# hammershock/SFM-Python

Hardware: AMD Instinct MI355X
Metric: BA iterations/sec (higher is better)
Workload: dtype f64

## Files before the change

### sfm-python_amd/csrc/ba_kernels.hpp

```cpp
#pragma once

#include <hip/hip_runtime.h>
#include <stdint.h>

#include "tr2d.hpp"

namespace sfmba {

constexpr int kCamTab = 17;
constexpr int kCamRow = 18;
#ifndef SFMBA_REC_LAYOUT
#define SFMBA_REC_LAYOUT 0
#endif
constexpr int kRecLayout = SFMBA_REC_LAYOUT;
constexpr int kRec = kRecLayout == 0 ? 6 : (kRecLayout == 1 ? 8 : 16);
constexpr int kVinvRow = kRecLayout == 0 ? 6 : (kRecLayout == 1 ? 8 : 16);
constexpr int kVinvInRec = kRecLayout == 2 ? 8 : -1;
constexpr int kRhsRec = 16;
constexpr int kSweepThreads = 1024;
constexpr int kWavesPerSweepBlock = kSweepThreads / 64;

struct KMat { double k[9]; };

constexpr int kJPlanes = 6;
// ... 1026 lines not shown
                }
            }
#pragma unroll
            for (int u = 0; u < kScalePts; ++u) {
                const int p = p0 + u * (int)blockDim.x;
                if (p >= P) continue;
#pragma unroll
                for (int k = 0; k < 3; ++k) {
                    double s, sge;
                    element(d[u][k], ge[u][k], so[u][k], xe[u][k], s, sge);
                    sip[(size_t)p * 3 + k] = s; gpo[(size_t)p * 3 + k] = ge[u][k]; sgp[(size_t)p * 3 + k] = sge;
                }
            }
        }
    }
    write_partials(q, part);
}


__global__ void k_post(Mailbox mb) { post_mailbox(mb); }

__global__ void k_finish(const double* __restrict__ part, FinishJob job, int nq, int first_sum,
                         double* __restrict__ out, const double* __restrict__ skip, Mailbox mb) {
    if (skip != nullptr && *skip != 0.0) {
        if (mb.host != nullptr && blockIdx.x == 0 && threadIdx.x < 64) post_mailbox(mb);
        return;
    }
    const int k = threadIdx.x >> 6;
    if (k < nq) finish_task(part, job, (int)blockIdx.x, k, nq, first_sum, out);
    if (mb.host != nullptr) {
        __syncthreads();
        if (threadIdx.x < 64) post_mailbox(mb);
    }
}

struct Recompute {
    const double* __restrict__ camtab;
    const double* __restrict__ pts;
    KMat K;
};
__device__ __forceinline__ void stage_cam_table(const double* __restrict__ camtab, int C, double* __restrict__ smem) {
    const int n2 = (C * kCamRow) >> 1;
    const double2* __restrict__ src = reinterpret_cast<const double2*>(camtab);
    double2* __restrict__ dst = reinterpret_cast<double2*>(smem);
    for (int k = threadIdx.x; k < n2; k += blockDim.x) dst[k] = src[k];
    __syncthreads();
}
__device__ __forceinline__ void recompute_blocks(const Recompute& rc, const double* __restrict__ tab_lds, int c, int p,
                                                 double* jc, double* jp) {
    double tl[kCamRow];
    const double2* __restrict__ trow = reinterpret_cast<const double2*>(tab_lds + (size_t)c * kCamRow);
#pragma unroll
    for (int k = 0; k < kCamRow / 2; ++k) { const double2 q = trow[k]; tl[2 * k] = q.x; tl[2 * k + 1] = q.y; }
    const double* __restrict__ Xp = rc.pts + 3 * (size_t)p;
    double rx, ry;
    observe<true>(tl, Xp[0], Xp[1], Xp[2], 0.0, 0.0, rc.K, rx, ry, jc, jp);
}

template <bool LDS_VEC, bool JFREE = false>
__global__ __launch_bounds__(kSweepThreads) void k_jdot(ObsArrays o, const double* __restrict__ sgc,
                                                        const double* __restrict__ sgp, int N, int C,
                                                        double* __restrict__ t1,
                                                        double* __restrict__ part, Piggyback pb, Recompute rc) {
    static_assert(!(LDS_VEC && JFREE), "J-free: the LDS holds the camera table, the vector comes from L2");
    extern __shared__ __align__(16) double smem[];
    __shared__ double red[kWavesPerSweepBlock];
// ... 2398 lines not shown
```

### sfm-python_amd/csrc/sfmba.hip

```cpp
#include "../../include/sfmba.h"

#include <hip/hip_runtime.h>
#include <hip/hip_ext.h>
#include <rccl/rccl.h>
#include <dlfcn.h>

#include <algorithm>
#include <atomic>
#include <chrono>
#include <cmath>
#include <cstdarg>
#include <cstdio>
#include <cstdlib>
#include <cstring>
#include <condition_variable>
#include <functional>
#include <mutex>
#include <numeric>
#include <string>
#include <thread>
#include <vector>

#include "ba_kernels.hpp"
#include "tr2d.hpp"
// ... 13 lines not shown
    void* p = nullptr;
    size_t bytes = 0;
    ~DevBuf() { if (p) (void)hipFree(p); }
    hipError_t ensure(size_t n) {
        if (n <= bytes && p) return hipSuccess;
        if (p) { (void)hipFree(p); p = nullptr; bytes = 0; }
        if (n == 0) n = 8;
        hipError_t e = hipMalloc(&p, n);
        if (e == hipSuccess) bytes = n;
        return e;
    }
    hipError_t ensure_keep(size_t n, size_t keep) {
        if (n <= bytes && p) return hipSuccess;
        if (keep == 0 || !p) return ensure(n + n / 2);
        void* q = nullptr;
        const size_t cap = n + n / 2;
        hipError_t e = hipMalloc(&q, cap);
        if (e != hipSuccess) return e;
        e = hipMemcpy(q, p, std::min(keep, bytes), hipMemcpyDeviceToDevice);
        (void)hipFree(p);
        p = q; bytes = cap;
        return e;
    }
    template <class T> T* as() const { return static_cast<T*>(p); }
};

struct DevView {
    void* p = nullptr;
    template <class T> T* as() const { return static_cast<T*>(p); }
};

struct PinnedBuf {
    void* p = nullptr;
    size_t bytes = 0;
    ~PinnedBuf() { if (p) (void)hipHostFree(p); }
    hipError_t ensure(size_t n, size_t keep) {
        if (n <= bytes && p) return hipSuccess;
        void* q = nullptr;
        const size_t cap = n + n / 2 + 64;
        hipError_t e = hipHostMalloc(&q, cap, hipHostMallocDefault);
        if (e != hipSuccess) return e;
        if (p && keep) memcpy(q, p, std::min(keep, bytes));
        if (p) (void)hipHostFree(p);
        p = q; bytes = cap;
        return hipSuccess;
    }
    template <class T> T* as() const { return static_cast<T*>(p); }
};

class HostPool {
public:
    static constexpr int kMax = 16;
    ~HostPool() {
        { std::lock_guard<std::mutex> lk(m_); stop_ = true; ++gen_; }
        cv_.notify_all();
        for (auto& t : th_) t.join();
    }
    int parts_for(int64_t n) const {
        const int hw = (int)std::thread::hardware_concurrency();
        return (int)std::max<int64_t>(1, std::min<int64_t>(std::min(kMax, hw > 0 ? hw : 1), n / 65536));
    }
    template <class Fn>
    void run(int parts, Fn fn) {
        if (parts <= 1) { fn(0); return; }
        while ((int)th_.size() < parts - 1) {
            const int id = (int)th_.size() + 1;
            th_.emplace_back([this, id] { worker(id); });
        }
        std::function<void(int)> f = fn;
        {
            std::lock_guard<std::mutex> lk(m_);
            job_ = &f; job_parts_ = parts; pending_ = parts - 1; ++gen_;
        }
        cv_.notify_all();
        fn(0);
        std::unique_lock<std::mutex> lk(m_);
        done_.wait(lk, [this] { return pending_ == 0; });
        job_ = nullptr;
    }
private:
    void worker(int id) {
        unsigned long long seen = 0;
        for (;;) {
            std::function<void(int)>* f = nullptr;
            {
                std::unique_lock<std::mutex> lk(m_);
                cv_.wait(lk, [&] { return gen_ != seen; });
                seen = gen_;
                if (stop_) return;
                if (id >= job_parts_ || job_ == nullptr) continue;
                f = job_;
            }
            (*f)(id);
            {
                std::lock_guard<std::mutex> lk(m_);
                if (--pending_ == 0) done_.notify_one();
            }
        }
    }
    std::vector<std::thread> th_;
    std::mutex m_;
    std::condition_variable cv_, done_;
    std::function<void(int)>* job_ = nullptr;
    int job_parts_ = 0, pending_ = 0;
    unsigned long long gen_ = 0;
    bool stop_ = false;
};

struct RcclApi {
    void* lib = nullptr;
    ncclResult_t (*GetUniqueId)(ncclUniqueId*) = nullptr;
    ncclResult_t (*CommInitRank)(ncclComm_t*, int, ncclUniqueId, int) = nullptr;
    ncclResult_t (*AllReduce)(const void*, void*, size_t, ncclDataType_t, ncclRedOp_t, ncclComm_t, hipStream_t) = nullptr;
    ncclResult_t (*CommDestroy)(ncclComm_t) = nullptr;
    const char* (*GetErrorString)(ncclResult_t) = nullptr;
};
RcclApi* rccl_api() {
    static RcclApi api;
    static bool tried = false;
    if (!tried) {
        tried = true;
        void* lib = dlopen("librccl.so.1", RTLD_NOW | RTLD_GLOBAL);
        if (!lib) lib = dlopen("librccl.so", RTLD_NOW | RTLD_GLOBAL);
        if (!lib) lib = dlopen("/opt/rocm/lib/librccl.so.1", RTLD_NOW | RTLD_GLOBAL);
        if (lib) {
            api.GetUniqueId = (decltype(api.GetUniqueId))dlsym(lib, "ncclGetUniqueId");
            api.CommInitRank = (decltype(api.CommInitRank))dlsym(lib, "ncclCommInitRank");
            api.AllReduce = (decltype(api.AllReduce))dlsym(lib, "ncclAllReduce");
            api.CommDestroy = (decltype(api.CommDestroy))dlsym(lib, "ncclCommDestroy");
            api.GetErrorString = (decltype(api.GetErrorString))dlsym(lib, "ncclGetErrorString");
            if (api.GetUniqueId && api.CommInitRank && api.AllReduce && api.CommDestroy && api.GetErrorString)
                api.lib = lib;
        }
    }
    return api.lib ? &api : nullptr;
}

double now_s() {
    return std::chrono::duration<double>(std::chrono::steady_clock::now().time_since_epoch()).count();
// ... 25 lines not shown
    DevBuf rctab;
    bool jfree = false;
    bool mixed = false;
    bool mixed_b = false;
    DevBuf rt32, rec32, rctab32, rtd;
    Origin origin{0.0, 0.0, 0.0};
    bool dense = false;
    DevView cov_ptr, cov_pt, blk_ab;
    DevBuf Sblk;
    DevBuf tables;
    int n_blk = 0;
    struct Debug {
        int pcg_fused = -1;
        int tab_lds = -1, vec_lds = -1;
        int sweep_rc = -1;
        int dense = -1;
        int precond = -1;
        int pcg_local = -1;
        int xcd_chunks = -1;
        int rhsrec = -1;
        int cost_rider = -1;
        int packed_upload = -1;
        int jfree = -1;
        int cm_device = -1;
        int pcg_inline = -1;
        int xcd_cam = -1;
        int pcg_skip_last = -1;
        int pcg_mixed_b = -1;
        int pcg_mixed = -1;
        int pcg_split = -1;
        int spec_scale = -1;
        int start_handoff = -1;
        int early_download = -1;
        int cam_chunk = 0;
        int pcg_guess_bias = 0;
        int trace_pcg = 0, trace_stalls = 0, trace_timing = 0;
        int wait_deadline_s = 120;
        int p2p_delay_ms = 0;
        int p2p_timeout_ms = 0;
    } dbg;

    DevBuf cam_idx, pt_idx, pt_ptr, uv;
    DevView ranges, wsteps, steps;
    int n_steps = 0;
    DevBuf cm_perm, cm_pt, cm_uv, cam_partial;
    DevBuf sort_hist, fixed_dev;
    DevView cam_ptr_dev;
    DevView cam_chunks, cam_chunk_ptr;
    int n_chunks = 0;
    DevView cam_chunks_b, cam_chunk_ptr_b;
    int n_chunks_b = 0;
    bool xcd_b = false;
    std::vector<int4> host_chunks_b;
    std::vector<int> host_chunk_ptr_b;
    bool cam_multi = false;
    DevBuf xa, xb, tabA, tabB, r, J, t1;
    DevBuf rhsrec;
    DevBuf V, Vinv, gp, e, recA, recB;
    DevBuf edge;
    DevBuf g, si, sg, p;
    DevBuf g2, si2, sg2;
    DevBuf Dc, Minv, vecs, vtmp, vcm;
    DevBuf part, ctrl;
    DevBuf arena_own;
    double* arena = nullptr;
    int64_t arena_doubles = 0;
// ... 5 lines not shown
    int64_t n_collectives = 0, n_launches = 0;
    struct P2p {
        bool ready = false;
        int rank = 0, world = 0;
        int64_t stride = 0;
        void* own = nullptr;
        void* opened[kP2pMaxRanks] = {};
        double* data[kP2pMaxRanks] = {};
        unsigned long long* flags[kP2pMaxRanks] = {};
        double* camdata[kP2pMaxRanks] = {};
        unsigned* words = nullptr;
        int64_t calls = 0;
        bool first_in_solve = true;
        int shared_device = 1;
        bool any_multi = false;
    } p2p;
    double* h_scal = nullptr;
    struct Stage { PinnedBuf uv, ci, pi, perm, ptr, uvf, tables, ci16, uv16; } stage;
    DevBuf ci16_dev, uv16_dev;
    struct Prev { bool valid = false; bool f32 = false; bool packed = false; int64_t N = 0, P = 0; } prev;
    std::vector<int2> host_ranges, host_wsteps, host_steps;
    std::vector<int4> host_chunks;
    std::vector<int> host_chunk_ptr;
    HostPool pool;
    int64_t obs_reused = 0, obs_uploaded = 0;
    double* mbox = nullptr;
    double* mbox_dev = nullptr;
    unsigned long long mbox_seq = 0;
    Mailbox post{};
    double* h_x = nullptr;
    size_t h_x_doubles = 0;
    hipStream_t copy_stream = nullptr;
    hipEvent_t ev_written = nullptr, ev_copied[2] = {nullptr, nullptr};
    bool result_in_flight = false;
    PinnedBuf mirror[2];
    unsigned long long mirror_tag[2] = {0, 0}, copy_count = 0, x_tag = 0;
    bool mirror_on = false;
    const double* skip = nullptr;
    double pcg_tol = 0.0; int pcg_cap = 0;
    bool pcg_fused = false;
    bool pcg_local = false;
    bool pcg_local2 = false;
    bool pcg_b_owed = false;
    bool pcg_a_owed = false;
    bool pcg_inline = false;
    bool pcg_split = false;
    DevBuf pcg_part;
    int pcg_hint = 0;
    std::vector<int> pcg_hist;
    int64_t hist_C = 0, hist_P = 0, hist_N = 0;
    unsigned long long hist_sig = 0;
    unsigned long long problem_gen = 0;
    bool use_rhsrec = false;
    bool solved = false;
    bool transport_dropped = false;
    std::vector<const void*> lds_ready;
    int last_pcg_iters = 0;

    double* x = nullptr;
    double* x_new = nullptr;
    double* tab = nullptr;
    double* tab_new = nullptr;
    double* rec = nullptr;
    double* rec_new = nullptr;
    double* g_cur = nullptr;
    double* si_cur = nullptr;
// ... 728 lines not shown
    return pb;
}
int launch_finish_backsub(sfmba_handle* h, int nparts) {
    const Piggyback pb = backsub_rider(h, nparts);
    hipLaunchKernelGGL(k_finish, dim3(1), dim3(64 * kBacksubCols), 0, h->stream, pb.part, pb.job, kBacksubCols, 0,
                       h->scal(), (const double*)nullptr, Mailbox{});
    LAUNCHED(h);
    return 0;
}

int flush_scale_sums(sfmba_handle* h) {
    if (!h->pending_scale_sums) return 0;
    h->pending_scale_sums = false;
    return launch_finish_slices(h, 0, 4);
}
int exchange_linearise(sfmba_handle* h) {
    CHK(exchange(h, h->scal() + 8, 4, 0));
    CHK(exchange(h, h->scal() + kMaxSlot, 1, 1));
    return 0;
}
int exchange_tail(sfmba_handle* h) {
    return exchange(h, h->scal() + 2, 6, 0);
}

int fetch_scalars(sfmba_handle* h) {
    const Mailbox mb{h->mbox_dev, h->scal(), nullptr, ++h->mbox_seq, p2p_error_word(h)};
    hipLaunchKernelGGL(k_post, dim3(1), dim3(64), 0, h->stream, mb);
    LAUNCHED(h);
    CHK(wait_mailbox(h, h->mbox_seq));
    memcpy(h->h_scal, h->mbox, sizeof(double) * kScalSlots);
    return 0;
}

double qsum(const sfmba_handle* h, int q) { return h->h_scal[kPointSlot[q]] + h->h_scal[kCamSlot + q]; }

int ensure_h_x(sfmba_handle* h) {
    const size_t need = (size_t)std::max<int64_t>(h->n, 2 * h->N);
    if (h->h_x && h->h_x_doubles >= need) return 0;
    if (h->h_x) { (void)hipHostFree(h->h_x); h->h_x = nullptr; h->h_x_doubles = 0; }
    HIPCHK(h, hipHostMalloc((void**)&h->h_x, sizeof(double) * need, hipHostMallocDefault));
    h->h_x_doubles = need;
    return 0;
}

template <class Fn>
void staging_copy(sfmba_handle* h, void* dst, const void* src, size_t bytes, Fn chunk_done) {
    const int parts = (int)std::min<size_t>(4, bytes >> 19);
    if (parts <= 1) { memcpy(dst, src, bytes); chunk_done(0, (size_t)0, bytes); return; }
    const size_t per = ((bytes + parts - 1) / parts + 63) & ~(size_t)63;
    std::atomic<int> done[8];
    for (auto& d : done) d.store(0, std::memory_order_relaxed);
    h->pool.run(parts, [&](int t) {
        const size_t b = std::min(bytes, (size_t)t * per), e = std::min(bytes, b + per);
        if (e > b) memcpy(static_cast<char*>(dst) + b, static_cast<const char*>(src) + b, e - b);
        if (t != 0) { done[t].store(1, std::memory_order_release); return; }
        chunk_done(0, b, e - b);
        for (int k = 1; k < parts; ++k) {
            while (done[k].load(std::memory_order_acquire) == 0) { }
            const size_t bk = std::min(bytes, (size_t)k * per), ek = std::min(bytes, bk + per);
            chunk_done(k, bk, ek - bk);
        }
    });
}
void staging_copy(sfmba_handle* h, void* dst, const void* src, size_t bytes) {
    staging_copy(h, dst, src, bytes, [](int, size_t, size_t) {});
}

int upload_x(sfmba_handle* h, const double* x_host) {
    CHK(ensure_h_x(h));
    if (h->mixed) {
        const double* pts = x_host + 6 * h->C;
        const int64_t stride = std::max<int64_t>(1, h->P / 1024);
        double sx = 0.0, sy = 0.0, sz = 0.0;
        int64_t cnt = 0;
        for (int64_t q = 0; q < h->P; q += stride, ++cnt) { sx += pts[3 * q]; sy += pts[3 * q + 1]; sz += pts[3 * q + 2]; }
        h->origin = Origin{sx / (double)cnt, sy / (double)cnt, sz / (double)cnt};
        if (!std::isfinite(h->origin.x + h->origin.y + h->origin.z)) h->origin = Origin{0.0, 0.0, 0.0};
    }
    HIPCHK(h, hipStreamSynchronize(h->stream));
    if (h->result_in_flight && h->copy_stream) HIPCHK(h, hipStreamSynchronize(h->copy_stream));
    h->result_in_flight = false;
    const double t0 = now_s();
    hipError_t err = hipSuccess;
    staging_copy(h, h->h_x, x_host, sizeof(double) * h->n, [&](int, size_t off, size_t bytes) {
        if (bytes == 0 || err != hipSuccess) return;
        err = hipMemcpyAsync(reinterpret_cast<char*>(h->x) + off, reinterpret_cast<const char*>(h->h_x) + off, bytes,
                             hipMemcpyHostToDevice, h->stream);
    });
    HIPCHK(h, err);
    if (h->dbg.trace_timing) fprintf(stderr, "sfmba: upload_x  staging copy + enqueue %.1f us\n", 1e6 * (now_s() - t0));
    return 0;
}

int download_residuals(sfmba_handle* h, double* r_out) {
    CHK(ensure_h_x(h));
    HIPCHK(h, hipStreamSynchronize(h->stream));
    const size_t bytes = (h->f32 ? sizeof(float) : sizeof(double)) * 2 * (size_t)h->N;
    HIPCHK(h, hipMemcpyAsync(h->h_x, h->r.p, bytes, hipMemcpyDeviceToHost, h->stream));
// ... 192 lines not shown

int sfmba_create(sfmba_handle** out, int device_id) {
    if (!out) return -1;
    *out = nullptr;
    int ndev = 0;
    hipError_t e = hipGetDeviceCount(&ndev);
    if (e != hipSuccess || ndev <= 0) return -3;
    if (device_id < 0 || device_id >= ndev) return -1;
    auto* h = new sfmba_handle();
    h->device = device_id;
    if (hipSetDevice(device_id) != hipSuccess) { delete h; return -3; }
    hipDeviceProp_t prop;
    if (hipGetDeviceProperties(&prop, device_id) == hipSuccess) h->n_cu = prop.multiProcessorCount;
    if (hipStreamCreateWithFlags(&h->stream, hipStreamNonBlocking) != hipSuccess) { delete h; return -3; }
    h->own_stream = true;
    if (hipHostMalloc((void**)&h->h_scal, sizeof(double) * 64, hipHostMallocDefault) != hipSuccess ||
        hipHostMalloc((void**)&h->mbox, sizeof(double) * 64, hipHostMallocCoherent | hipHostMallocMapped) != hipSuccess ||
        hipHostGetDevicePointer((void**)&h->mbox_dev, h->mbox, 0) != hipSuccess) {
        (void)hipStreamDestroy(h->stream); delete h; return -4;
    }
    memset(h->mbox, 0, sizeof(double) * 64);
    {
        int prio_low = 0, prio_high = 0;
        if (hipDeviceGetStreamPriorityRange(&prio_low, &prio_high) != hipSuccess) prio_low = 0;
        if (hipStreamCreateWithPriority(&h->copy_stream, hipStreamNonBlocking, prio_low) != hipSuccess) h->copy_stream = nullptr;
    }
    if (h->copy_stream &&
        (hipEventCreateWithFlags(&h->ev_written, hipEventDisableTiming) != hipSuccess ||
         hipEventCreateWithFlags(&h->ev_copied[0], hipEventDisableTiming) != hipSuccess ||
         hipEventCreateWithFlags(&h->ev_copied[1], hipEventDisableTiming) != hipSuccess)) {
        (void)hipStreamDestroy(h->copy_stream);
        h->copy_stream = nullptr;
    }
    *out = h;
    return 0;
}

void sfmba_destroy(sfmba_handle* h) {
    if (!h) return;
    (void)hipSetDevice(h->device);
    if (h->stream) (void)hipStreamSynchronize(h->stream);
    if (h->comm) { if (RcclApi* api = rccl_api()) (void)api->CommDestroy(h->comm); h->comm = nullptr; }
    p2p_release(h);
    if (h->copy_stream) { (void)hipStreamSynchronize(h->copy_stream); (void)hipStreamDestroy(h->copy_stream); }
    if (h->ev_written) (void)hipEventDestroy(h->ev_written);
    for (auto& ev : h->ev_copied) if (ev) (void)hipEventDestroy(ev);
    if (h->own_stream && h->stream) (void)hipStreamDestroy(h->stream);
    if (h->h_scal) (void)hipHostFree(h->h_scal);
    if (h->mbox) (void)hipHostFree(h->mbox);
    if (h->h_x) (void)hipHostFree(h->h_x);
    delete h;
}

const char* sfmba_last_error(const sfmba_handle* h) { return h ? h->err.c_str() : "null handle"; }

int sfmba_set_stream(sfmba_handle* h, void* hip_stream) {
    CHK(enter(h));
    if (h->stream) HIPCHK(h, hipStreamSynchronize(h->stream));
    if (h->own_stream && h->stream) (void)hipStreamDestroy(h->stream);
    h->stream = static_cast<hipStream_t>(hip_stream);
    h->own_stream = false;
    return 0;
}

int sfmba_set_print(sfmba_handle* h, sfmba_print_fn fn, void* ctx) {
    CHK(enter(h));
    h->print_fn = fn;
    h->print_ctx = ctx;
    return 0;
}

int sfmba_debug_option(sfmba_handle* h, const char* name, int64_t value) {
    CHK(enter(h));
    if (!name) return fail(h, -1, "option name is NULL");
    const std::string n(name);
    const int v = (int)value;
    if (n == "pcg_fused") h->dbg.pcg_fused = v;
    else if (n == "sweep_rc") h->dbg.sweep_rc = v;
    else if (n == "dense") h->dbg.dense = v;
    else if (n == "precond") h->dbg.precond = v;
    else if (n == "pcg_local") h->dbg.pcg_local = v;
    else if (n == "pcg_split") h->dbg.pcg_split = v;
    else if (n == "pcg_mixed") h->dbg.pcg_mixed = v;
    else if (n == "pcg_inline") h->dbg.pcg_inline = v;
    else if (n == "pcg_skip_last") h->dbg.pcg_skip_last = v;
    else if (n == "xcd_cam") h->dbg.xcd_cam = v;
    else if (n == "cm_device") h->dbg.cm_device = v;
    else if (n == "jfree") h->dbg.jfree = v;
    else if (n == "packed_upload") h->dbg.packed_upload = v;
    else if (n == "pcg_mixed_b") h->dbg.pcg_mixed_b = v;
    else if (n == "cost_rider") h->dbg.cost_rider = v;
    else if (n == "spec_scale") h->dbg.spec_scale = v;
    else if (n == "start_handoff") h->dbg.start_handoff = v;
    else if (n == "early_download") h->dbg.early_download = v;
    else if (n == "rhsrec") h->dbg.rhsrec = v;
    else if (n == "xcd_chunks") h->dbg.xcd_chunks = v;
    else if (n == "tab_lds") h->dbg.tab_lds = v;
    else if (n == "vec_lds") h->dbg.vec_lds = v;
    else if (n == "cam_chunk") h->dbg.cam_chunk = v;
    else if (n == "pcg_guess_bias") h->dbg.pcg_guess_bias = v;
    else if (n == "trace_pcg") h->dbg.trace_pcg = v;
    else if (n == "trace_stalls") h->dbg.trace_stalls = v;
    else if (n == "trace_timing") h->dbg.trace_timing = v;
    else if (n == "wait_deadline_s") h->dbg.wait_deadline_s = v;
    else if (n == "p2p_delay_ms") h->dbg.p2p_delay_ms = v;
    else if (n == "p2p_timeout_ms") h->dbg.p2p_timeout_ms = v;
    else return fail(h, -1, "unknown debug option '%s'", name);
    return 0;
}

int sfmba_set_precision(sfmba_handle* h, int32_t storage_bits) {
    CHK(enter(h));
    if (storage_bits != 64 && storage_bits != 32) return fail(h, -1, "storage_bits must be 64 or 32");
    h->f32_next = storage_bits == 32;
    return 0;
}

int sfmba_set_fixed_cameras(sfmba_handle* h, const int64_t* camera_indices, int64_t n_fixed) {
    CHK(enter(h));
    if (n_fixed < 0 || (n_fixed > 0 && !camera_indices)) return fail(h, -1, "bad fixed-camera list");
    h->fixed_next.assign(camera_indices, camera_indices + n_fixed);
    return 0;
}

int64_t sfmba_exchange_doubles(int64_t n_cameras) { return 54 * n_cameras + kScalSlots; }

int sfmba_set_exchange(sfmba_handle* h, void* arena, int64_t arena_doubles, sfmba_allreduce_fn fn,
// ... 913 lines not shown
                hipLaunchKernelGGL((k_cam_rhs_diag<false>), dim3(h->n_chunks), dim3(kRhsThreads), 0, h->stream, cam_major(h),
                                   (const double*)h->tab, (const double*)h->rec, (const double*)vinv_ptr(h), h->K, (int)h->C,
                                   h->acc(), h->cam_partial.as<double>(), RhsPrecond{nullptr, nullptr, nullptr},
                                   h->use_rhsrec ? (const double*)h->rhsrec.as<double>() : (const double*)nullptr, CamExchange{});
                LAUNCHED(h);
                break;
            case 10:
                hipLaunchKernelGGL(k_fill16, dim3(h->n_cu * 2), dim3(1024), 0, h->stream, h->J.as<double>(),
                                   (int64_t)((h->f32 ? 3 : 6) * h->ld), 1.0);
                break;
            default: return fail(h, -1, "unknown kernel id %d", which);
        }
    }
    HIPCHK(h, hipEventRecord(ev.b, h->stream));
    HIPCHK(h, hipEventSynchronize(ev.b));
    float ms = 0.f;
    HIPCHK(h, hipEventElapsedTime(&ms, ev.a, ev.b));
    *avg_us = 1e3 * (double)ms / reps;
    HIPCHK(h, hipStreamSynchronize(h->stream));
    return 0;
}

static int solve_impl(sfmba_handle* h, const double* x_start, double* x_inout, const sfmba_options* opt_in, sfmba_result* out);

int sfmba_solve(sfmba_handle* h, double* x_inout, const sfmba_options* opt_in, sfmba_result* out) {
    return sfmba_solve_from(h, x_inout, x_inout, opt_in, out);
}

int sfmba_solve_from(sfmba_handle* h, const double* x0, double* x_out, const sfmba_options* opt_in, sfmba_result* out) {
    const int rc = solve_impl(h, x0, x_out, opt_in, out);
    if (rc != 0 && h) {
        const std::string msg = h->err;
        h->skip = nullptr; h->post = Mailbox{};
        if (h->stream) (void)hipStreamSynchronize(h->stream);
        if (h->copy_stream) (void)hipStreamSynchronize(h->copy_stream);
        if (rc == -5 && h->p2p.ready) {
            p2p_close_peers(h);
            if (h->p2p.words) (void)hipMemset(h->p2p.words, 0, 4 * sizeof(unsigned));
        }
        h->err = msg;
    }
    return rc;
}

static int solve_impl(sfmba_handle* h, const double* x_start, double* x_inout, const sfmba_options* opt_in, sfmba_result* out) {
    CHK(enter(h));
    CHK(check_ready(h, x_start));
    if (!x_inout) return fail(h, -1, "x_out is NULL");
    if (!out) return fail(h, -1, "result is NULL");
    sfmba_options opt;
    if (opt_in) opt = *opt_in; else sfmba_default_options(&opt);
    memset(out, 0, sizeof *out);
    h->solved = false;
    h->skip = nullptr; h->post = Mailbox{};
    h->pending_scale_sums = false;
    h->p2p.first_in_solve = true;
    if (h->dbg.p2p_delay_ms > 0) std::this_thread::sleep_for(std::chrono::milliseconds(h->dbg.p2p_delay_ms));
    const double t_begin = now_s();
    const int64_t C = h->C, P = h->P, n = h->n;
    const int64_t max_nfev = opt.max_nfev > 0 ? opt.max_nfev : 100 * (6 * C + 3 * P);
    const double m_total = 2.0 * (double)h->N_total;
    double* sc = h->scal();

    h->x = h->xa.as<double>(); h->x_new = h->xb.as<double>();
    h->tab = h->tabA.as<double>(); h->tab_new = h->tabB.as<double>();
    h->rec = h->recA.as<double>(); h->rec_new = h->recB.as<double>();
    CHK(upload_x(h, x_start));
    h->mirror_on = h->copy_stream != nullptr && n >= 2000000;
    h->x_tag = 0; h->mirror_tag[0] = h->mirror_tag[1] = 0;
    if (h->mirror_on) {
        HIPCHK(h, h->mirror[0].ensure(sizeof(double) * n, 0));
        HIPCHK(h, h->mirror[1].ensure(sizeof(double) * n, 0));
    }
    HIPCHK(h, hipMemsetAsync(h->scal() + kGhPrevSlot, 0, 2 * sizeof(double), h->stream));
    const double t_dev0 = now_s();
    report_stall(h, "upload_x", t_dev0 - t_begin);

    struct EventList : std::vector<std::pair<hipEvent_t, hipEvent_t>> {
        ~EventList() { for (auto& pr : *this) { (void)hipEventDestroy(pr.first); (void)hipEventDestroy(pr.second); } }
    } evs;
    int np_cost = 0;
    const bool quick_start = !multi_rank(h) && h->dbg.start_handoff != 0 && h->dbg.cost_rider != 0;
    const bool spec_scale = !multi_rank(h) && h->dbg.spec_scale != 0;
    const bool early_download = h->copy_stream != nullptr && h->dbg.early_download != 0;
    bool result_sent = false;
    double t_sent0 = 0.0, t_sent1 = 0.0, t_ws = 0.0;
    auto eval_jac = [&](const double* x, double* tab, bool table_ready, bool finish = true) -> int {
        if (!table_ready) CHK(launch_cam_table(h, x, tab, h->rec, quick_start));
        int& np = np_cost;
        if (opt.profile) {
            hipEvent_t a, b;
            HIPCHK(h, hipEventCreateWithFlags(&a, hipEventDisableSystemFence));
            if (hipEventCreateWithFlags(&b, hipEventDisableSystemFence) != hipSuccess) {
                (void)hipEventDestroy(a);
                return fail(h, -3, "hipEventCreateWithFlags failed");
            }
            evs.emplace_back(a, b);
            CHK((launch_resjac<true, true>(h, x, tab, &np, a, b)));
        } else {
            CHK((launch_resjac<true, true>(h, x, tab, &np)));
        }
        if (finish) CHK(launch_finish(h, h->part.as<double>(), np, 1, 0));
        return 0;
    };
    auto linearise = [&](int first) -> int {
        CHK(launch_normal_blocks(h, h->x, h->tab, h->rec));
// ... 29 lines not shown
    int64_t nfev = 1, njev = 1, iteration = 0, pcg_total = 0;
    int status = -1;
    double step_norm = 0.0, actual_reduction = 0.0, g_norm = 0.0, reg_term = 0.0;
    bool have_red = false;
    int pcg_guess = h->pcg_hint;
    std::vector<int> pcg_hist_new;
    bool guess_exact = false;
    unsigned long long sig = h->problem_gen * 0x9E3779B97F4A7C15ull;
    {
        const int64_t stride = std::max<int64_t>(1, n / 509);
        for (int64_t k = 0; k < n; k += stride) {
            unsigned long long bits;
            memcpy(&bits, x_start + k, sizeof bits);
            sig = (sig ^ bits) * 0x100000001B3ull;
        }
    }
    const bool hist_same = h->hist_C == C && h->hist_P == P && h->hist_N == h->N && h->hist_sig == sig;
    const bool hist_near = hist_same || (h->hist_N > 0 && std::llabs(h->hist_C - C) <= 1 && 2 * h->N >= h->hist_N && h->N <= 2 * h->hist_N);
    if (!hist_near) { h->pcg_hist.clear(); h->pcg_hint = 0; pcg_guess = 0; }
    if (!h->pcg_hist.empty() && h->pcg_hist[0] > 0) { pcg_guess = h->pcg_hist[0]; guess_exact = hist_same; }
    int64_t pcg_breakdowns = 0;
    bool nb_valid = true;
    const bool pcg_debug = h->dbg.trace_pcg != 0;
    const int pcg_bias = h->dbg.pcg_guess_bias;
    if (opt.verbose >= 2) print_header(h);

    for (;;) {
        if (!nb_valid) {
            CHK(eval_jac(h->x, h->tab, true));
            CHK(launch_normal_blocks(h, h->x, h->tab, h->rec));
            nb_valid = true;
        }
        const bool one_rank = !multi_rank(h);
        int np = 0;
        const bool scale_sums_rode = h->pending_scale_sums;
        CHK(launch_jdot(h, &np));
        if (start_seq != 0) {
            CHK(wait_mailbox(h, start_seq));
            memcpy(h->h_scal, h->mbox, sizeof(double) * kScalSlots);
            start_seq = 0;
            CHK(start_values());
        }
        if (!one_rank && h->p2p.ready) {
            Piggyback pb{h->partB(), sc, FinishJob{}, 1, 1, 0};
            pb.job.row0[0] = 0; pb.job.nrows[0] = np;
            for (int k = 0; k < kNQ; ++k) { pb.job.slot[0][k] = 1 + k; pb.job.slot[1][k] = -1; }
            static_assert(kMaxSlot == 12, "mask below assumes the maximum sits at the end of the run");
            CHK(p2p_allreduce(h, sc + 1, scale_sums_rode ? kMaxSlot : 1, 0, nullptr,
                              scale_sums_rode ? 1ull << (kMaxSlot - 1) : 0ull, &pb));
            ++h->n_collectives;
        } else if (!one_rank) {
            CHK(launch_finish(h, h->partB(), np, 1, 1));
            if (scale_sums_rode) CHK(exchange_linearise(h));
            CHK(exchange(h, sc + 1, 1, 0));
        }
        {
            const int bc = (int)((C + 63) / 64), bp = (int)((P + 63) / 64);
            hipLaunchKernelGGL(k_prep, dim3(bc + bp), dim3(64), 0, h->stream, sc, Delta, opt.reg_min, h->Ugc(),
                               h->V.as<double>(), h->gp.as<double>(), h->si_cur, (int)C, (int)P, bc,
                               h->Dc.as<double>(), (h->dbg.precond == 0 ? h->Minv.as<double>() : (double*)nullptr),
                               vinv_ptr(h), h->rec + 3,
                               one_rank ? (const double*)h->partB() : (const double*)nullptr, np, opt.pcg_tol,
                               std::max(opt.pcg_tol, opt.pcg_tol_max), (const double*)(h->x + 6 * C),
                               (h->use_rhsrec && !(h->dense && one_rank)) ? h->rhsrec.as<double>() : (double*)nullptr,
                               (h->dense && one_rank) ? MixedPrep{nullptr, nullptr, nullptr, nullptr, Origin{0.0, 0.0, 0.0}} : mixed_prep(h, h->tab));
            LAUNCHED(h);
// ... 10 lines not shown
            CHK(pcg_finish_polling(h, opt, &hc));
        }
        int np_tail = 0;
        auto tail = [&](bool for_device_step) -> int {
            CHK(launch_backsub(h, &np));
            np_tail = np;
            if (!one_rank && h->p2p.ready) {
                const Piggyback pb = backsub_rider(h, np);
                CHK(p2p_allreduce(h, sc + 2, 6, 0, nullptr, 0, &pb));
                ++h->n_collectives;
                return 0;
            }
            if (!(for_device_step && one_rank)) CHK(launch_finish_backsub(h, np));
            CHK(exchange_tail(h));
            return 0;
        };
        CHK(tail(true));

        Mailbox trial_post{};
        bool trial_post_pending = false;
        auto enqueue_trial = [&](const double* coef_dev, double c1, double c2) -> int {
            const int bc = (int)((C + 255) / 256);
            hipLaunchKernelGGL(k_step_table, dim3(bc + grid_1d(3 * P, 256, 2048)), dim3(256), 0, h->stream, h->x,
                               h->sg_cur, h->p.as<double>(), c1, c2, coef_dev, (int)C, n, bc, h->x_new,
                               h->tab_new, h->rec_new, h->skip);
            LAUNCHED(h);
            if (h->mirror_on) {
                const int w = h->x_new == h->xa.as<double>() ? 0 : 1;
                HIPCHK(h, hipEventRecord(h->ev_written, h->stream));
                HIPCHK(h, hipStreamWaitEvent(h->copy_stream, h->ev_written, 0));
                HIPCHK(h, hipMemcpyAsync(h->mirror[w].p, h->x_new, sizeof(double) * n, hipMemcpyDeviceToHost, h->copy_stream));
                HIPCHK(h, hipEventRecord(h->ev_copied[w], h->copy_stream));
                h->mirror_tag[w] = ++h->copy_count;
            }
            const Mailbox mb{h->mbox_dev, sc, h->ctrl.as<PcgCtrl>() + (h->pcg_L & 1), ++h->mbox_seq, p2p_error_word(h)};
            const bool ranks = multi_rank(h);
            if (ranks && h->p2p.ready) {
                CHK(eval_jac(h->x_new, h->tab_new, true, false));
                Piggyback pb{h->part.as<double>(), sc, FinishJob{}, 1, 1, 0};
                pb.job.row0[0] = 0; pb.job.nrows[0] = np_cost;
                for (int k = 0; k < kNQ; ++k) { pb.job.slot[0][k] = k; pb.job.slot[1][k] = -1; }
                CHK(p2p_allreduce(h, sc, 1, 0, nullptr, 0, &pb, &mb, h->skip));
                ++h->n_collectives;
                return 0;
            }
            if (!ranks && h->dbg.cost_rider == 0) {
                h->post = mb;
                const int rc = eval_jac(h->x_new, h->tab_new, true);
                h->post = Mailbox{};
                return rc;
            }
            if (!ranks) {
                CHK(eval_jac(h->x_new, h->tab_new, true, false));
                trial_post = mb;
                trial_post_pending = true;
                return 0;
            }
            CHK(eval_jac(h->x_new, h->tab_new, true));
            CHK(exchange(h, sc, 1, 0));
            hipLaunchKernelGGL(k_post, dim3(1), dim3(64), 0, h->stream, mb);
            LAUNCHED(h);
            return 0;
        };
        auto handoff = [&](bool with_ctrl) -> int {
            if (trial_post_pending) CHK(launch_normal_blocks(h, h->x_new, h->tab_new, h->rec_new, np_cost, trial_post));
            else CHK(launch_normal_blocks(h, h->x_new, h->tab_new, h->rec_new));
            trial_post_pending = false;
            nb_valid = false;
            if (spec_scale) CHK(launch_update_scale(h, 0, true, true));
            CHK(wait_mailbox(h, h->mbox_seq));
            memcpy(h->h_scal, h->mbox, sizeof(double) * kScalSlots);
            if (with_ctrl) memcpy(&hc, h->mbox + kMboxCtrl, sizeof hc);
            return 0;
        };
        const bool speculated = pcg_guess > 0 || dense;
        const int pcg_enqueued = pcg_guess > 0 ? pcg_guess + (h->pcg_fused ? 1 : 0) + (guess_exact ? 0 : 1) : 0;
        bool missed = false;
        for (bool speculative = speculated;;) {
            hipLaunchKernelGGL(k_tr_step, dim3(1), dim3(one_rank ? 1024 : 64), 0, h->stream, sc, Delta,
                               speculative ? (const PcgCtrl*)(h->ctrl.as<PcgCtrl>() + (h->pcg_L & 1)) : (const PcgCtrl*)nullptr,
                               one_rank ? backsub_rider(h, np_tail) : Piggyback{});
            LAUNCHED(h);
            h->skip = sc + 30;
            int rc_trial = enqueue_trial(sc + 25, 0.0, 0.0);
            if (rc_trial == 0) rc_trial = handoff(speculative);
            h->skip = nullptr;
            CHK(rc_trial);
            if (!(speculative && hc.done == 0)) break;
            missed = true;
            nb_valid = true;
            if (opt.profile && !evs.empty()) {
                (void)hipEventDestroy(evs.back().first);
                (void)hipEventDestroy(evs.back().second);
                evs.pop_back();
            }
            CHK(pcg_finish_polling(h, opt, &hc));
            CHK(tail(true));
            speculative = false;
        }
        bool first_trial_ready = true;
        if (hc.done == 3) ++pcg_breakdowns;
        if (Delta < 0.0) Delta = h->h_scal[31];
// ... 29 lines not shown
            if (first_trial_ready) {
                st.c1 = h->h_scal[25]; st.c2 = h->h_scal[26]; st.predicted = h->h_scal[27];
                st.step_h_norm = h->h_scal[28]; st.step_norm = h->h_scal[29];
                first_trial_ready = false;
            } else {
                st = tr_solve_step(model, Delta);
                CHK(enqueue_trial(nullptr, st.c1, st.c2));
                CHK(handoff(false));
            }
            ++nfev;
            cost_new = 0.5 * h->h_scal[0];
            if (!std::isfinite(cost_new)) {
                Delta = 0.25 * st.step_h_norm;
                continue;
            }
            actual_reduction = cost - cost_new;
            double ratio;
            const double Delta_new = update_tr_radius(Delta, actual_reduction, st.predicted, st.step_h_norm,
                                                      st.step_h_norm > 0.95 * Delta, &ratio);
            step_norm = st.step_norm;
            const int term = check_termination(actual_reduction, cost, step_norm, x_norm, ratio, opt.ftol, opt.xtol);
            if (term != 0) { status = term; break; }
            Delta = Delta_new;
        }
        have_red = true;
        if (actual_reduction > 0.0) {
            std::swap(h->x, h->x_new);
            std::swap(h->tab, h->tab_new);
            std::swap(h->rec, h->rec_new);
            h->x_tag = h->mirror_tag[h->x == h->xa.as<double>() ? 0 : 1];
            nb_valid = true;
            cost = cost_new;
            ++njev;
            if (status != -1 && early_download && !h->mirror_on) {
                CHK(ensure_h_x(h));
                t_sent0 = now_s();
                HIPCHK(h, hipMemcpyAsync(h->h_x, h->x, sizeof(double) * (size_t)n, hipMemcpyDeviceToHost, h->copy_stream));
                HIPCHK(h, hipEventRecord(h->ev_copied[0], h->copy_stream));
                h->result_in_flight = true;
                result_sent = true;
                t_sent1 = now_s();
            }
            if (spec_scale) {
                std::swap(h->g_cur, h->g_new);
                std::swap(h->si_cur, h->si_new);
                std::swap(h->sg_cur, h->sg_new);
                h->pending_scale_sums = true;
            } else {
                CHK(launch_update_scale(h, 0, true));
            }
        } else {
            step_norm = 0.0;
            actual_reduction = 0.0;
        }
        ++iteration;
        if (status != -1) {
            if (h->pending_scale_sums) {
                CHK(flush_scale_sums(h));
                CHK(exchange_linearise(h));
            }
            CHK(fetch_scalars(h));
            g_norm = std::max(h->h_scal[kMaxSlot], h->h_scal[kCamSlot + 0]);
            if (opt.verbose >= 2) print_iter(h, iteration, nfev, cost, have_red, actual_reduction, step_norm, g_norm);
            break;
        }
    }
    if (status == -1) status = 0;
    if (!nb_valid) {
        int np = 0;
        CHK((launch_resjac<false, true>(h, h->x, h->tab, &np)));
    }

    CHK(ensure_h_x(h));
    const double t_dl0 = now_s();
    const int xw = h->x == h->xa.as<double>() ? 0 : 1;
    const bool mirrored = h->mirror_on && h->x_tag != 0 && h->mirror_tag[xw] == h->x_tag;
    const size_t xbytes = sizeof(double) * (size_t)n;
    if (!mirrored && !result_sent) {
        HIPCHK(h, hipMemcpyAsync(h->h_x, h->x, xbytes, hipMemcpyDeviceToHost, h->stream));
    }
    if (h->p2p.ready)
        HIPCHK(h, hipMemcpyAsync(h->h_scal + 62, h->p2p.words + 1, sizeof(unsigned), hipMemcpyDeviceToHost, h->stream));
    CHK(wait_stream(h));
    t_ws = now_s();
    if (result_sent) {
        CHK(wait_event(h, h->ev_copied[0]));
        h->result_in_flight = false;
    }
    if (mirrored) HIPCHK(h, hipEventSynchronize(h->ev_copied[xw]));
    const double t_dl1 = now_s();
    if (h->p2p.ready) {
        unsigned err = 0;
        memcpy(&err, h->h_scal + 62, sizeof err);
        if (err != 0) return p2p_timed_out(h, err);
    }
    staging_copy(h, x_inout, mirrored ? h->mirror[xw].p : (const void*)h->h_x, xbytes);
    if (h->mirror_on) HIPCHK(h, hipStreamSynchronize(h->copy_stream));
    const double t_end = now_s();
    if (h->dbg.trace_timing && result_sent)
        fprintf(stderr, "sfmba: early result copy: enqueue %.1f us, then %.1f us to the last post, stream query %.1f us, copy event %.1f us\n",
                1e6 * (t_sent1 - t_sent0), 1e6 * (t_dl0 - t_sent1), 1e6 * (t_ws - t_dl0), 1e6 * (t_dl1 - t_ws));
    if (h->dbg.trace_timing)
        fprintf(stderr, "sfmba: solve  %.3f ms total, upload %.1f us, result: copy + wait %.1f us, staging copy %.1f us\n", 1e3 * (t_end - t_begin),
                1e6 * (t_dev0 - t_begin), 1e6 * (t_dl1 - t_dl0), 1e6 * (t_end - t_dl1));
    if (!evs.empty()) {
        double tot = 0.0;
        for (auto& pr : evs) {
            float ms = 0.f;
            if (hipEventElapsedTime(&ms, pr.first, pr.second) == hipSuccess) tot += ms;
        }
        out->resjac_avg_us = 1e3 * tot / (double)evs.size();
        out->resjac_launches = (int64_t)evs.size();
    }
    h->pcg_hist.swap(pcg_hist_new);
    h->hist_C = C; h->hist_P = P; h->hist_N = h->N; h->hist_sig = sig;
    out->cost = cost;
    out->optimality = g_norm;
    out->rmse = std::sqrt(2.0 * cost / m_total);
    out->nfev = nfev; out->njev = njev; out->iterations = iteration; out->pcg_iterations = pcg_total;
    out->status = status;
    out->seconds_total = t_end - t_begin;
    out->seconds_device = t_end - t_dev0;
    out->last_step_norm = step_norm;
    out->last_reg = reg_term;
    out->reserved = (int32_t)pcg_breakdowns;
    h->solved = true;
    return 0;
}

int sfmba_get_fun_grad(sfmba_handle* h, double* fun_out, double* grad_out) {
    CHK(enter(h));
// ... 17 lines not shown
```

Measured before the change: 2696.

## Speculatively mirror trial points to mapped host memory and stage results concurrently

```diff
diff --git a/sfm-python_amd/csrc/ba_kernels.hpp b/sfm-python_amd/csrc/ba_kernels.hpp
--- a/sfm-python_amd/csrc/ba_kernels.hpp
+++ b/sfm-python_amd/csrc/ba_kernels.hpp
@@ -1082,6 +1082,37 @@
         __syncthreads();
         if (threadIdx.x < 64) post_mailbox(mb);
     }
+}
+
+__global__ void __launch_bounds__(64 * kNQ) k_finish_post(const double* __restrict__ part, FinishJob job, int first_sum,
+                                                          double* __restrict__ out, Mailbox mb) {
+    const int k = threadIdx.x >> 6;
+    finish_task(part, job, 0, k, kNQ, first_sum, out);
+    finish_task(part, job, 1, k, kNQ, first_sum, out);
+    __syncthreads();
+    if (threadIdx.x < 64) post_mailbox(mb);
+}
+
+__device__ __forceinline__ void post_arrival(unsigned long long* __restrict__ word, unsigned long long value) {
+    __threadfence_system();
+    __hip_atomic_store(word, value, __ATOMIC_RELAXED, __HIP_MEMORY_SCOPE_SYSTEM);
+}
+__global__ void __launch_bounds__(256) k_copy_out(const double* __restrict__ src, double* __restrict__ dst, int64_t count,
+                                                  unsigned long long* __restrict__ arrive, unsigned long long value) {
+    if (arrive != nullptr && blockIdx.x == 0 && threadIdx.x == 0) post_arrival(arrive, value);
+    const double2* __restrict__ s2 = reinterpret_cast<const double2*>(src);
+    double2* __restrict__ d2 = reinterpret_cast<double2*>(dst);
+    const int64_t n2 = count >> 1, stride = (int64_t)gridDim.x * 256;
+    int64_t k = (int64_t)blockIdx.x * 256 + threadIdx.x;
+    for (; k + 3 * stride < n2; k += 4 * stride) {
+        const double2 a = s2[k], b = s2[k + stride], c = s2[k + 2 * stride], d = s2[k + 3 * stride];
+        d2[k] = a; d2[k + stride] = b; d2[k + 2 * stride] = c; d2[k + 3 * stride] = d;
+    }
+    for (; k < n2; k += stride) d2[k] = s2[k];
+    if ((count & 1) != 0 && blockIdx.x == 0 && threadIdx.x == 0) dst[count - 1] = src[count - 1];
+}
+__global__ void k_arrive(unsigned long long* __restrict__ word, unsigned long long value) {
+    if (threadIdx.x == 0) post_arrival(word, value);
 }
 
 struct Recompute {
diff --git a/sfm-python_amd/csrc/sfmba.hip b/sfm-python_amd/csrc/sfmba.hip
--- a/sfm-python_amd/csrc/sfmba.hip
+++ b/sfm-python_amd/csrc/sfmba.hip
@@ -69,17 +69,20 @@
 
 struct PinnedBuf {
     void* p = nullptr;
+    void* dev = nullptr;
     size_t bytes = 0;
     ~PinnedBuf() { if (p) (void)hipHostFree(p); }
-    hipError_t ensure(size_t n, size_t keep) {
-        if (n <= bytes && p) return hipSuccess;
+    hipError_t ensure(size_t n, size_t keep, bool mapped = false) {
+        if (n <= bytes && p && (!mapped || dev)) return hipSuccess;
         void* q = nullptr;
+        void* qd = nullptr;
         const size_t cap = n + n / 2 + 64;
-        hipError_t e = hipHostMalloc(&q, cap, hipHostMallocDefault);
+        hipError_t e = hipHostMalloc(&q, cap, mapped ? (hipHostMallocCoherent | hipHostMallocMapped) : hipHostMallocDefault);
         if (e != hipSuccess) return e;
+        if (mapped && (e = hipHostGetDevicePointer(&qd, q, 0)) != hipSuccess) { (void)hipHostFree(q); return e; }
         if (p && keep) memcpy(q, p, std::min(keep, bytes));
         if (p) (void)hipHostFree(p);
-        p = q; bytes = cap;
+        p = q; dev = qd; bytes = cap;
         return hipSuccess;
     }
     template <class T> T* as() const { return static_cast<T*>(p); }
@@ -142,6 +145,94 @@
     int job_parts_ = 0, pending_ = 0;
     unsigned long long gen_ = 0;
     bool stop_ = false;
+};
+
+class Stager {
+public:
+    static constexpr int kPieces = 4;
+    struct Job {
+        const char* src = nullptr;
+        char* dst = nullptr;
+        size_t per = 0, bytes = 0;
+        int parts = 0;
+        const unsigned long long* words = nullptr;
+        unsigned long long tag = 0;
+        double t_submit = 0.0;
+    };
+    static constexpr int kWordStride = 8;
+    ~Stager() {
+        cancel_join();
+        { std::lock_guard<std::mutex> lk(m_); stop_ = true; ++gen_; }
+        cv_.notify_all();
+        for (auto& t : th_) t.join();
+    }
+    void submit(const Job& job) {
+        cancel_join();
+        while ((int)th_.size() < job.parts) {
+            const int id = (int)th_.size();
+            th_.emplace_back([this, id] { worker(id); });
+        }
+        cancel_.store(0, std::memory_order_relaxed);
+        skipped_.store(0, std::memory_order_relaxed);
+        pending_.store(job.parts, std::memory_order_relaxed);
+        { std::lock_guard<std::mutex> lk(m_); job_ = job; ++gen_; }
+        cv_.notify_all();
+    }
+    bool busy() const { return pending_.load(std::memory_order_acquire) != 0; }
+    bool join(double deadline_s) {
+        const double t0 = now();
+        for (int spin = 0; pending_.load(std::memory_order_acquire) != 0; ++spin) {
+            __builtin_ia32_pause();
+            if ((spin & 1023) == 1023 && now() - t0 > deadline_s) { cancel_join(); return false; }
+        }
+        return job_.parts > 0 && skipped_.load(std::memory_order_relaxed) == 0;
+    }
+    void cancel_join() {
+        cancel_.store(1, std::memory_order_release);
+        while (pending_.load(std::memory_order_acquire) != 0) __builtin_ia32_pause();
+    }
+    unsigned long long tag() const { return job_.tag; }
+    double t_arrived[kPieces] = {}, t_copied[kPieces] = {};
+private:
+    static double now() { return std::chrono::duration<double>(std::chrono::steady_clock::now().time_since_epoch()).count(); }
+    void worker(int id) {
+        unsigned long long seen = 0;
+        for (;;) {
+            Job j;
+            {
+                std::unique_lock<std::mutex> lk(m_);
+                cv_.wait(lk, [&] { return gen_ != seen; });
+                seen = gen_;
+                if (stop_) return;
+                if (id >= job_.parts) continue;
+                j = job_;
+            }
+            const unsigned long long* word = j.words + (size_t)id * kWordStride;
+            bool arrived = false;
+            for (int spin = 0;; ++spin) {
+                if (__atomic_load_n(word, __ATOMIC_ACQUIRE) == j.tag) { arrived = true; break; }
+                if (cancel_.load(std::memory_order_acquire) != 0) break;
+                __builtin_ia32_pause();
+                if (spin > (1 << 16)) std::this_thread::yield();
+            }
+            if (arrived) {
+                t_arrived[id] = 1e6 * (now() - j.t_submit);
+                const size_t b = std::min(j.bytes, (size_t)id * j.per), e = std::min(j.bytes, b + j.per);
+                if (e > b) memcpy(j.dst + b, j.src + b, e - b);
+                t_copied[id] = 1e6 * (now() - j.t_submit);
+            } else {
+                skipped_.fetch_add(1, std::memory_order_relaxed);
+            }
+            pending_.fetch_sub(1, std::memory_order_release);
+        }
+    }
+    std::vector<std::thread> th_;
+    std::mutex m_;
+    std::condition_variable cv_;
+    Job job_;
+    unsigned long long gen_ = 0;
+    bool stop_ = false;
+    std::atomic<int> cancel_{0}, skipped_{0}, pending_{0};
 };
 
 struct RcclApi {
@@ -233,6 +324,9 @@
         int spec_scale = -1;
         int start_handoff = -1;
         int early_download = -1;
+        int spec_result = -1;
+        int copy_grid = 0;
+        int mirror_min = -1;
         int cam_chunk = 0;
         int pcg_guess_bias = 0;
         int trace_pcg = 0, trace_stalls = 0, trace_timing = 0;
@@ -304,6 +398,10 @@
     size_t h_x_doubles = 0;
     hipStream_t copy_stream = nullptr;
     hipEvent_t ev_written = nullptr, ev_copied[2] = {nullptr, nullptr};
+    bool spec_on = false;
+    unsigned long long* arrive = nullptr;
+    unsigned long long* arrive_dev = nullptr;
+    Stager stager;
     bool result_in_flight = false;
     PinnedBuf mirror[2];
     unsigned long long mirror_tag[2] = {0, 0}, copy_count = 0, x_tag = 0;
@@ -1098,6 +1196,17 @@
     return 0;
 }
 
+int finish_slices_and_fetch(sfmba_handle* h) {
+    h->pending_scale_sums = false;
+    const Mailbox mb{h->mbox_dev, h->scal(), nullptr, ++h->mbox_seq, p2p_error_word(h)};
+    hipLaunchKernelGGL(k_finish_post, dim3(1), dim3(64 * kNQ), 0, h->stream, (const double*)h->part.as<double>(),
+                       slices_job(h, 0, 4), 1, h->scal(), mb);
+    LAUNCHED(h);
+    CHK(wait_mailbox(h, h->mbox_seq));
+    memcpy(h->h_scal, h->mbox, sizeof(double) * kScalSlots);
+    return 0;
+}
+
 double qsum(const sfmba_handle* h, int q) { return h->h_scal[kPointSlot[q]] + h->h_scal[kCamSlot + q]; }
 
 int ensure_h_x(sfmba_handle* h) {
@@ -1130,6 +1239,56 @@
 }
 void staging_copy(sfmba_handle* h, void* dst, const void* src, size_t bytes) {
     staging_copy(h, dst, src, bytes, [](int, size_t, size_t) {});
+}
+
+constexpr int64_t kMirrorMinParams = 131072;
+constexpr size_t kCopyKernelMaxBytes = (size_t)16 << 20;
+constexpr int kCopyGrid = 16;
+struct Pieces { int parts; size_t per, bytes; };
+Pieces result_pieces(const sfmba_handle* h) {
+    const size_t bytes = sizeof(double) * (size_t)h->n;
+    const int parts = (int)std::max<size_t>(1, std::min<size_t>(Stager::kPieces, bytes >> 19));
+    return Pieces{parts, ((bytes + parts - 1) / parts + 63) & ~(size_t)63, bytes};
+}
+unsigned long long* arrival_words(const sfmba_handle* h, int w, bool dev) {
+    return (dev ? h->arrive_dev : h->arrive) + (size_t)w * Stager::kPieces * Stager::kWordStride;
+}
+
+int launch_mirror_copy(sfmba_handle* h, int w, unsigned long long tag) {
+    const Pieces pc = result_pieces(h);
+    unsigned long long* words = arrival_words(h, w, true);
+    const bool by_kernel = pc.bytes < kCopyKernelMaxBytes;
+    const int grid = h->dbg.copy_grid > 0 ? std::min(h->dbg.copy_grid, 1024) : kCopyGrid;
+    HIPCHK(h, hipStreamWaitEvent(h->copy_stream, h->ev_written, 0));
+    for (int k = 0; k < pc.parts; ++k) {
+        const size_t b = std::min(pc.bytes, (size_t)k * pc.per), e = std::min(pc.bytes, b + pc.per);
+        const double* src = h->x_new + b / sizeof(double);
+        if (by_kernel) {
+            hipLaunchKernelGGL(k_copy_out, dim3(grid), dim3(256), 0, h->copy_stream, src,
+                               static_cast<double*>(h->mirror[w].dev) + b / sizeof(double), (int64_t)((e - b) / sizeof(double)),
+                               k > 0 ? words + (size_t)(k - 1) * Stager::kWordStride : (unsigned long long*)nullptr, tag);
+            LAUNCHED(h);
+            if (k + 1 < pc.parts) continue;
+        } else if (e > b) {
+            HIPCHK(h, hipMemcpyAsync(static_cast<char*>(h->mirror[w].p) + b, src, e - b, hipMemcpyDeviceToHost, h->copy_stream));
+        }
+        hipLaunchKernelGGL(k_arrive, dim3(1), dim3(64), 0, h->copy_stream, words + (size_t)k * Stager::kWordStride, tag);
+        LAUNCHED(h);
+    }
+    return 0;
+}
+
+int wait_mirror(sfmba_handle* h, int w, unsigned long long tag) {
+    const Pieces pc = result_pieces(h);
+    const unsigned long long* words = arrival_words(h, w, false);
+    const double t0 = now_s();
+    for (int k = 0; k < pc.parts; ++k)
+        for (int spin = 0; __atomic_load_n(words + (size_t)k * Stager::kWordStride, __ATOMIC_ACQUIRE) != tag; ++spin) {
+            __builtin_ia32_pause();
+            if ((spin & 1023) == 1023 && now_s() - t0 > h->dbg.wait_deadline_s)
+                return fail(h, -3, "result mirror not complete within %d s: the device queue is stuck", h->dbg.wait_deadline_s);
+        }
+    return 0;
 }
 
 int upload_x(sfmba_handle* h, const double* x_host) {
@@ -1388,6 +1547,15 @@
         (void)hipStreamDestroy(h->copy_stream);
         h->copy_stream = nullptr;
     }
+    {
+        const size_t bytes = sizeof(unsigned long long) * 2 * Stager::kPieces * Stager::kWordStride;
+        if (hipHostMalloc((void**)&h->arrive, bytes, hipHostMallocCoherent | hipHostMallocMapped) != hipSuccess) h->arrive = nullptr;
+        if (h->arrive && hipHostGetDevicePointer((void**)&h->arrive_dev, h->arrive, 0) != hipSuccess) {
+            (void)hipHostFree(h->arrive);
+            h->arrive = nullptr;
+        }
+        if (h->arrive) memset(h->arrive, 0, bytes);
+    }
     *out = h;
     return 0;
 }
@@ -1395,6 +1563,7 @@
 void sfmba_destroy(sfmba_handle* h) {
     if (!h) return;
     (void)hipSetDevice(h->device);
+    h->stager.cancel_join();
     if (h->stream) (void)hipStreamSynchronize(h->stream);
     if (h->comm) { if (RcclApi* api = rccl_api()) (void)api->CommDestroy(h->comm); h->comm = nullptr; }
     p2p_release(h);
@@ -1404,6 +1573,7 @@
     if (h->own_stream && h->stream) (void)hipStreamDestroy(h->stream);
     if (h->h_scal) (void)hipHostFree(h->h_scal);
     if (h->mbox) (void)hipHostFree(h->mbox);
+    if (h->arrive) (void)hipHostFree(h->arrive);
     if (h->h_x) (void)hipHostFree(h->h_x);
     delete h;
 }
@@ -1449,6 +1619,9 @@
     else if (n == "spec_scale") h->dbg.spec_scale = v;
     else if (n == "start_handoff") h->dbg.start_handoff = v;
     else if (n == "early_download") h->dbg.early_download = v;
+    else if (n == "spec_result") h->dbg.spec_result = v;
+    else if (n == "copy_grid") h->dbg.copy_grid = v;
+    else if (n == "mirror_min") h->dbg.mirror_min = v;
     else if (n == "rhsrec") h->dbg.rhsrec = v;
     else if (n == "xcd_chunks") h->dbg.xcd_chunks = v;
     else if (n == "tab_lds") h->dbg.tab_lds = v;
@@ -2428,6 +2601,7 @@
     if (rc != 0 && h) {
         const std::string msg = h->err;
         h->skip = nullptr; h->post = Mailbox{};
+        h->stager.cancel_join();
         if (h->stream) (void)hipStreamSynchronize(h->stream);
         if (h->copy_stream) (void)hipStreamSynchronize(h->copy_stream);
         if (rc == -5 && h->p2p.ready) {
@@ -2462,12 +2636,18 @@
     h->tab = h->tabA.as<double>(); h->tab_new = h->tabB.as<double>();
     h->rec = h->recA.as<double>(); h->rec_new = h->recB.as<double>();
     CHK(upload_x(h, x_start));
-    h->mirror_on = h->copy_stream != nullptr && n >= 2000000;
+    h->spec_on = h->copy_stream != nullptr && h->arrive != nullptr && !multi_rank(h) && h->dbg.spec_result != 0 &&
+                 n >= (h->dbg.mirror_min >= 0 ? (int64_t)h->dbg.mirror_min : kMirrorMinParams);
+    h->mirror_on = !h->spec_on && h->copy_stream != nullptr && n >= 2000000;
     h->x_tag = 0; h->mirror_tag[0] = h->mirror_tag[1] = 0;
-    if (h->mirror_on) {
-        HIPCHK(h, h->mirror[0].ensure(sizeof(double) * n, 0));
-        HIPCHK(h, h->mirror[1].ensure(sizeof(double) * n, 0));
-    }
+    if (h->mirror_on || h->spec_on) {
+        HIPCHK(h, h->mirror[0].ensure(sizeof(double) * n, 0, h->spec_on));
+        HIPCHK(h, h->mirror[1].ensure(sizeof(double) * n, 0, h->spec_on));
+    }
+    const bool spec_out = h->spec_on && std::thread::hardware_concurrency() >= 8 &&
+                          (x_inout + n <= x_start || x_start + n <= x_inout);
+    bool mirror_pending = false;
+    int spec_trials = 0;
     HIPCHK(h, hipMemsetAsync(h->scal() + kGhPrevSlot, 0, 2 * sizeof(double), h->stream));
     const double t_dev0 = now_s();
     report_stall(h, "upload_x", t_dev0 - t_begin);
@@ -2563,6 +2743,7 @@
             nb_valid = true;
         }
         const bool one_rank = !multi_rank(h);
+        const bool last_pass = nfev >= max_nfev || (opt.max_iter > 0 && iteration >= opt.max_iter);
         int np = 0;
         const bool scale_sums_rode = h->pending_scale_sums;
         CHK(launch_jdot(h, &np));
@@ -2639,6 +2820,14 @@
                 HIPCHK(h, hipMemcpyAsync(h->mirror[w].p, h->x_new, sizeof(double) * n, hipMemcpyDeviceToHost, h->copy_stream));
                 HIPCHK(h, hipEventRecord(h->ev_copied[w], h->copy_stream));
                 h->mirror_tag[w] = ++h->copy_count;
+            }
+            if (h->spec_on) {
+                const int w = h->x_new == h->xa.as<double>() ? 0 : 1;
+                h->mirror_tag[w] = 0;
+                if (!last_pass) {
+                    HIPCHK(h, hipEventRecord(h->ev_written, h->stream));
+                    mirror_pending = true;
+                }
             }
             const Mailbox mb{h->mbox_dev, sc, h->ctrl.as<PcgCtrl>() + (h->pcg_L & 1), ++h->mbox_seq, p2p_error_word(h)};
             const bool ranks = multi_rank(h);
@@ -2675,6 +2864,25 @@
             trial_post_pending = false;
             nb_valid = false;
             if (spec_scale) CHK(launch_update_scale(h, 0, true, true));
+            if (mirror_pending) {
+                mirror_pending = false;
+                const int w = h->x_new == h->xa.as<double>() ? 0 : 1;
+                if (spec_out) h->stager.cancel_join();
+                h->mirror_tag[w] = ++h->copy_count;
+                CHK(launch_mirror_copy(h, w, h->mirror_tag[w]));
+                if (spec_out) {
+                    const Pieces pc = result_pieces(h);
+                    Stager::Job job;
+                    job.src = static_cast<const char*>(h->mirror[w].p);
+                    job.dst = reinterpret_cast<char*>(x_inout);
+                    job.per = pc.per; job.bytes = pc.bytes; job.parts = pc.parts;
+                    job.words = arrival_words(h, w, false);
+                    job.tag = h->mirror_tag[w];
+                    job.t_submit = now_s();
+                    h->stager.submit(job);
+                }
+                ++spec_trials;
+            }
             CHK(wait_mailbox(h, h->mbox_seq));
             memcpy(h->h_scal, h->mbox, sizeof(double) * kScalSlots);
             if (with_ctrl) memcpy(&hc, h->mbox + kMboxCtrl, sizeof hc);
@@ -2770,7 +2978,7 @@
             nb_valid = true;
             cost = cost_new;
             ++njev;
-            if (status != -1 && early_download && !h->mirror_on) {
+            if (status != -1 && early_download && !h->mirror_on && !(h->spec_on && h->x_tag != 0)) {
                 CHK(ensure_h_x(h));
                 t_sent0 = now_s();
                 HIPCHK(h, hipMemcpyAsync(h->h_x, h->x, sizeof(double) * (size_t)n, hipMemcpyDeviceToHost, h->copy_stream));
@@ -2793,11 +3001,15 @@
         }
         ++iteration;
         if (status != -1) {
-            if (h->pending_scale_sums) {
-                CHK(flush_scale_sums(h));
-                CHK(exchange_linearise(h));
+            if (h->pending_scale_sums && !multi_rank(h) && h->dbg.spec_result != 0) {
+                CHK(finish_slices_and_fetch(h));
+            } else {
+                if (h->pending_scale_sums) {
+                    CHK(flush_scale_sums(h));
+                    CHK(exchange_linearise(h));
+                }
+                CHK(fetch_scalars(h));
             }
-            CHK(fetch_scalars(h));
             g_norm = std::max(h->h_scal[kMaxSlot], h->h_scal[kCamSlot + 0]);
             if (opt.verbose >= 2) print_iter(h, iteration, nfev, cost, have_red, actual_reduction, step_norm, g_norm);
             break;
@@ -2812,8 +3024,10 @@
     CHK(ensure_h_x(h));
     const double t_dl0 = now_s();
     const int xw = h->x == h->xa.as<double>() ? 0 : 1;
-    const bool mirrored = h->mirror_on && h->x_tag != 0 && h->mirror_tag[xw] == h->x_tag;
+    const bool mirrored = (h->mirror_on || h->spec_on) && h->x_tag != 0 && h->mirror_tag[xw] == h->x_tag;
     const size_t xbytes = sizeof(double) * (size_t)n;
+    const bool staged_tag = spec_out && mirrored && h->stager.tag() == h->x_tag;
+    if (spec_out && !staged_tag) h->stager.cancel_join();
     if (!mirrored && !result_sent) {
         HIPCHK(h, hipMemcpyAsync(h->h_x, h->x, xbytes, hipMemcpyDeviceToHost, h->stream));
     }
@@ -2825,16 +3039,30 @@
         CHK(wait_event(h, h->ev_copied[0]));
         h->result_in_flight = false;
     }
-    if (mirrored) HIPCHK(h, hipEventSynchronize(h->ev_copied[xw]));
+    if (mirrored && h->mirror_on) HIPCHK(h, hipEventSynchronize(h->ev_copied[xw]));
+    bool staged = false;
+    if (staged_tag) staged = h->stager.join((double)h->dbg.wait_deadline_s);
+    if (mirrored && h->spec_on && !staged) CHK(wait_mirror(h, xw, h->x_tag));
     const double t_dl1 = now_s();
     if (h->p2p.ready) {
         unsigned err = 0;
         memcpy(&err, h->h_scal + 62, sizeof err);
         if (err != 0) return p2p_timed_out(h, err);
     }
-    staging_copy(h, x_inout, mirrored ? h->mirror[xw].p : (const void*)h->h_x, xbytes);
-    if (h->mirror_on) HIPCHK(h, hipStreamSynchronize(h->copy_stream));
+    if (!staged) staging_copy(h, x_inout, mirrored ? h->mirror[xw].p : (const void*)h->h_x, xbytes);
+    if (h->mirror_on || (h->spec_on && h->copy_count != h->x_tag))
+        HIPCHK(h, hipStreamSynchronize(h->copy_stream));
     const double t_end = now_s();
+    if (h->dbg.trace_timing && h->spec_on) {
+        const Pieces pc = result_pieces(h);
+        fprintf(stderr, "sfmba: result overlap: %d trial points mirrored in %d pieces, result %s;", spec_trials, pc.parts,
+                staged ? "staged while the solve ran" : mirrored ? "in its mirror" : "copied behind the solve");
+        if (staged)
+            for (int k = 0; k < pc.parts; ++k)
+                fprintf(stderr, " piece %d arrived %.1f us after its submit, staged at %.1f us%s", k, h->stager.t_arrived[k],
+                        h->stager.t_copied[k], k + 1 < pc.parts ? "," : "");
+        fprintf(stderr, "\n");
+    }
     if (h->dbg.trace_timing && result_sent)
         fprintf(stderr, "sfmba: early result copy: enqueue %.1f us, then %.1f us to the last post, stream query %.1f us, copy event %.1f us\n",
                 1e6 * (t_sent1 - t_sent0), 1e6 * (t_dl0 - t_sent1), 1e6 * (t_ws - t_dl0), 1e6 * (t_dl1 - t_ws));
```

After: 2577. -4.4%, worse.
